# millardjn/rusty_sr

Measured on AMD Instinct MI355X. Metric: output megapixels/sec at 3x upscale (BASELINE '4x'; reference factor is hard-wired 3), higher is better.
Workload: dtype f32; 1 GPU; 1920x1080 RGB x3 upscale per GPU, imagenet.rsr, rgba8 in/out resident in HBM; io=rgba8, factor=3, parallelism=rowband1, precision=f32

## Files before the change

rusty_sr_amd/csrc/sr_kernels.hip:

```cpp
#include <hip/hip_runtime.h>
#include <stddef.h>
#include <stdint.h>

#include <mutex>
#include <set>
#include <type_traits>
#include <utility>

#include "sr_kernels.h"

#pragma clang fp contract(off)

typedef float f32x2 __attribute__((ext_vector_type(2)));
struct f32p { float x, y; };
__device__ __forceinline__ f32p operator+(f32p a, f32p b) { return f32p{a.x + b.x, a.y + b.y}; }
__device__ __forceinline__ f32p operator-(f32p a, f32p b) { return f32p{a.x - b.x, a.y - b.y}; }
__device__ __forceinline__ f32p operator*(f32p a, f32p b) { return f32p{a.x * b.x, a.y * b.y}; }
__device__ __forceinline__ f32p p_fma(f32p a, f32p b, f32p c) { return f32p{__builtin_fmaf(a.x, b.x, c.x), __builtin_fmaf(a.y, b.y, c.y)}; }
__device__ __forceinline__ void store_map8(char* p, uint32_t a, uint32_t b) { *(uint2*)p = make_uint2(a, b); }
typedef float f32x4 __attribute__((ext_vector_type(4)));
typedef float f32x16 __attribute__((ext_vector_type(16)));
typedef _Float16 f16x8 __attribute__((ext_vector_type(8)));
typedef _Float16 f16x2 __attribute__((ext_vector_type(2)));

template <int PREC>
constexpr bool kPlanar = PREC == 1;
template <int PREC, bool FINAL>
constexpr bool kH16 = PREC == 1 && !FINAL;

namespace {

constexpr int kThreads = 256;
constexpr int kTW = 32;
constexpr int kChunkFloats = 1024;
constexpr int kRingSlots = 5;
constexpr int kRingAhead = 4;
constexpr int kRingBytes = kRingSlots * 4096;

__device__ __forceinline__ float belu(float v, float beta) {
    return __fadd_rn(__fadd_rn(__fmul_rn(beta, v), __builtin_amdgcn_sqrtf(__fadd_rn(__fmul_rn(v, v), 1.0f))), -1.0f);
}

__device__ __forceinline__ f32x2 belu2(f32x2 v, float beta) {
    const f32x2 one = {1.0f, 1.0f};
    const f32x2 t = v * v + one;
    const f32x2 s = {__builtin_amdgcn_sqrtf(t.x), __builtin_amdgcn_sqrtf(t.y)};
    const f32x2 b = {beta, beta};
    return (b * v + s) - one;
}

__device__ __forceinline__ f32p split_value(f32p accm, f32p accx) {
    return p_fma(accx, f32p{1.0f / 2048.0f, 1.0f / 2048.0f}, accm);
}
__device__ __forceinline__ f32p belu2_fused2(f32p v, f32p beta) {
    const f32p one = {1.0f, 1.0f};
    const f32p t = p_fma(v, v, one);
    const f32p s = {__builtin_amdgcn_sqrtf(t.x), __builtin_amdgcn_sqrtf(t.y)};
    return p_fma(beta, v, s) - one;
}

__device__ __forceinline__ void store_belu_tile(float* base, const f32x16& acc, float bias, float beta) {
#pragma unroll
    for (int r = 0; r < 16; r += 2) {
        const f32x2 bb = {bias, bias};
        const f32x2 o = belu2(f32x2{acc[r], acc[r + 1]} + bb, beta);
        const int row = (r & 3) + 8 * (r >> 2);
        base[row * 32] = o.x;
        base[(row + 1) * 32] = o.y;
    }
}

__device__ __forceinline__ void store_belu_tile_lds(float* grow, float* stage, const f32x16& acc, float bias, float beta, int lane) {
    float* sp = stage + (4 * (lane >> 5)) * 32 + (lane & 31);
#pragma unroll
    for (int r = 0; r < 16; r += 2) {
        const f32x2 bb = {bias, bias};
        const f32x2 o = belu2(f32x2{acc[r], acc[r + 1]} + bb, beta);
        const int row = (r & 3) + 8 * (r >> 2);
        sp[row * 32] = o.x;
        sp[(row + 1) * 32] = o.y;
    }
    const f32x4* lp = (const f32x4*)stage + lane;
    const f32x4 v0 = lp[0], v1 = lp[64], v2 = lp[128], v3 = lp[192];
    f32x4* gp = (f32x4*)grow + lane;
    gp[0] = v0; gp[64] = v1; gp[128] = v2; gp[192] = v3;
}

__device__ __forceinline__ int xcd_remap(int bid, int nblk) {
    const int q = nblk >> 3, r = nblk & 7, xcd = bid & 7, idx = bid >> 3;
    return (xcd < r ? xcd * (q + 1) : r * (q + 1) + (xcd - r) * q) + idx;
}

__device__ __forceinline__ int tile_div(int t, TileDiv d) {
    return (int)((__umulhi((uint32_t)t, d.m) + (uint32_t)t) >> d.s);
}

__device__ __forceinline__ void tile_coords(const TileGrid& g, int tiles_x, int t, int& n, int& tx, int& ty) {
    const int tpi = tiles_x * g.tiles_y;
    n = tile_div(t, g.div_tpi);
    const int r = t - n * tpi;
    if (g.bw == 0) {
        ty = tile_div(r, g.div_tx);
        tx = r - ty * tiles_x;
    } else {
        int b = tile_div(r, g.div_blk);
        if (b > g.nfull) b = g.nfull;
        const int rr = r - b * g.bw * g.tiles_y;
        const bool full = b < g.nfull;
        const int w = full ? g.bw : tiles_x - g.nfull * g.bw;
        ty = full ? tile_div(rr, g.div_bw) : tile_div(rr, g.div_rem);
        tx = b * g.bw + (rr - ty * w);
    }
}

__device__ __forceinline__ float load_img(const void* img, int img_ch, bool u8, size_t px, int c) {
    if (u8) return __fdiv_rn((float)((const uint8_t*)img)[px * img_ch + c], 255.0f);
    return ((const float*)img)[px * 3 + c];
}

constexpr float kLoScale = 2048.0f;
typedef __fp16 fp16x2_t __attribute__((ext_vector_type(2)));

__device__ __forceinline__ void split_half2(f32p v, uint32_t& hi2, uint32_t& lo2) {
    const fp16x2_t h = __builtin_amdgcn_cvt_pkrtz(v.x, v.y);
    const f32p hf = {(float)h.x, (float)h.y};
    const f32p r = (v - hf) * f32p{kLoScale, kLoScale};
    hi2 = __builtin_bit_cast(uint32_t, h);
    lo2 = __builtin_bit_cast(uint32_t, __builtin_amdgcn_cvt_pkrtz(r.x, r.y));
}

typedef unsigned short u16x2 __attribute__((ext_vector_type(2)));
__device__ __forceinline__ void domain_track(uint32_t& dom, uint32_t hi2) {
    dom = __builtin_bit_cast(uint32_t, __builtin_elementwise_max(__builtin_bit_cast(u16x2, dom), __builtin_bit_cast(u16x2, hi2 & 0x7fff7fffu)));
}
__device__ __forceinline__ void domain_report(uint32_t dom, int* flag) {
    if (((dom & 0xffffu) >= 0x7bffu) | ((dom >> 16) >= 0x7bffu)) *(volatile int*)flag = 1;
}

__device__ __forceinline__ void store_belu_tile_split_cr(char* base, const f32x16& accm, const f32x16& accx, const f32x4 (&beta)[4], bool write,
                                                         long group_stride, long lo_off, uint32_t& dom) {
#pragma unroll
    for (int j = 0; j < 4; ++j) {
        const int r = 4 * j;
        const f32p v01 = belu2_fused2(split_value(f32p{accm[r], accm[r + 1]}, f32p{accx[r], accx[r + 1]}), f32p{beta[j][0], beta[j][1]});
        const f32p v23 = belu2_fused2(split_value(f32p{accm[r + 2], accm[r + 3]}, f32p{accx[r + 2], accx[r + 3]}), f32p{beta[j][2], beta[j][3]});
        uint32_t h01, l01, h23, l23;
        split_half2(v01, h01, l01);
        split_half2(v23, h23, l23);
        domain_track(dom, h01);
        domain_track(dom, h23);
        if (write) {
            store_map8(base + j * group_stride, h01, h23);
            store_map8(base + j * group_stride + lo_off, l01, l23);
        }
    }
}

template <typename F>
__device__ __forceinline__ void for_each_acc_row(F&& f) {
#pragma unroll
    for (int r = 0; r < 16; ++r) f(r, (r & 3) + 8 * (r >> 2));
}

}

__device__ __forceinline__ const char* uniform_ptr(const void* p) {
    const uint64_t v = (uint64_t)(uintptr_t)p;
    const uint32_t lo = __builtin_amdgcn_readfirstlane((uint32_t)v), hi = __builtin_amdgcn_readfirstlane((uint32_t)(v >> 32));
    return (const char*)(uintptr_t)(((uint64_t)hi << 32) | lo);
}

template <int TH, bool IMG_U8>
__global__ __launch_bounds__(kThreads, 2) void conv0_kernel(Conv0Args a) {
    constexpr int T = TH / 4;
    constexpr int TWH = kTW + 4, THH = TH + 4, NPIX = THH * TWH;
    __shared__ __attribute__((aligned(16))) float s_x[NPIX * 3 + 16];
    __shared__ __attribute__((aligned(16))) float s_w[5 * 8 * 64];

    const int tid = threadIdx.x, lane = tid & 63;
    const int wave = __builtin_amdgcn_readfirstlane(tid >> 6);
    const int i = lane & 31, h = lane >> 5;
    const int tiles_per_img = a.tiles_x * a.tiles_y;
    for (int k = tid; k < 5 * 8 * 64; k += kThreads) s_w[k] = a.wpack[k];
    if (tid < 16) s_x[NPIX * 3 + tid] = 0.f;
    if (blockIdx.x == 0 && tid < 40) a.queue_reset[tid] = (a.queue_grid[tid >> 3] - (tid & 7) + 7) >> 3;
    __shared__ float s_lut[256];
    if constexpr (IMG_U8) s_lut[tid] = __fdiv_rn((float)tid, 255.0f);
    const float bias = a.bias[i], beta = a.beta[i];
  for (int bid = blockIdx.x; bid < a.n_tiles; bid += gridDim.x) {
    const int n = tile_div(bid, a.div_tpi), t = bid - n * tiles_per_img;
    const int ty = tile_div(t, a.div_tx), tx = t - ty * a.tiles_x;
    const int x0 = tx * kTW, y0 = a.y_begin + ty * TH;
    const size_t img_px0 = (size_t)n * a.H * a.W;

    __syncthreads();
    for (int p = tid; p < NPIX; p += kThreads) {
        const int py = p / TWH, px = p - py * TWH;
        const int gy = y0 - 2 + py, gx = x0 - 2 + px;
        f32x4 v = {0.f, 0.f, 0.f, 0.f};
        if (gy >= 0 && gy < a.H && gx >= 0 && gx < a.W) {
            const size_t gp = img_px0 + (size_t)gy * a.W + gx;
            if constexpr (IMG_U8) {
                const uint8_t* q = (const uint8_t*)a.img + gp * a.img_ch;
                v.x = s_lut[q[0]]; v.y = s_lut[q[1]]; v.z = s_lut[q[2]];
            } else {
                v.x = load_img(a.img, a.img_ch, false, gp, 0);
                v.y = load_img(a.img, a.img_ch, false, gp, 1);
                v.z = load_img(a.img, a.img_ch, false, gp, 2);
            }
        }
        s_x[p * 3] = v.x; s_x[p * 3 + 1] = v.y; s_x[p * 3 + 2] = v.z;
    }
    __syncthreads();

    f32x16 acc[T];
#pragma unroll
    for (int m = 0; m < T; ++m)
#pragma unroll
        for (int r = 0; r < 16; ++r) acc[m][r] = 0.f;

    const float* xa = s_x + ((wave * T) * TWH + i) * 3 + h;
    const float* wb = s_w + (h * 32 + i) * 2;
#pragma unroll
    for (int ky = 0; ky < 5; ++ky) {
#pragma unroll
        for (int jj = 0; jj < 4; ++jj) {
            const f32x2 b = *(const f32x2*)(wb + (ky * 4 + jj) * 128);
#pragma unroll
            for (int m = 0; m < T; ++m) {
                const float* row = xa + (m + ky) * TWH * 3;
                acc[m] = __builtin_amdgcn_mfma_f32_32x32x2f32(row[4 * jj], b.x, acc[m], 0, 0, 0);
                const float a2 = (jj == 3 && h) ? 0.0f : row[4 * jj + 2];
                acc[m] = __builtin_amdgcn_mfma_f32_32x32x2f32(a2, b.y, acc[m], 0, 0, 0);
            }
        }
    }

    const bool full_x = x0 + kTW <= a.W;
#pragma unroll
    for (int m = 0; m < T; ++m) {
        const int y = y0 + wave * T + m;
        if (y >= a.y_end) continue;
        float* base = a.dst + ((size_t)n * a.img_stride + (long)y * a.pitch + x0 + 4 * h) * 32 + i;
        if (full_x) {
            store_belu_tile(base, acc[m], bias, beta);
        } else {
            for_each_acc_row([&](int r, int row) {
                if (x0 + 4 * h + row < a.W) base[row * 32] = belu(__fadd_rn(acc[m][r], bias), beta);
            });
        }
    }
  }
}

template <int TH, bool IMG_U8>
__global__ __launch_bounds__(kThreads, 3) void conv0_split_kernel(Conv0Args a) {
    constexpr int T = TH / 4;
    constexpr int TWH = kTW + 4, THH = TH + 4, NPIX = THH * TWH;
    constexpr int NB = 7;
    __shared__ __attribute__((aligned(16))) uint32_t s_px[2][NPIX * 2];
    __shared__ uint32_t s_lut[256];
    const int tid = threadIdx.x, lane = tid & 63;
    const int wave = __builtin_amdgcn_readfirstlane(tid >> 6);
    const int i = lane & 31, h = lane >> 5;
    const int tiles_per_img = a.tiles_x * a.tiles_y;
    if (blockIdx.x == 0 && tid < 40) a.queue_reset[tid] = (a.queue_grid[tid >> 3] - (tid & 7) + 7) >> 3;
    if constexpr (IMG_U8) {
        uint32_t hi2, lo2;
        split_half2(f32p{__fdiv_rn((float)tid, 255.0f), 0.0f}, hi2, lo2);
        s_lut[tid] = (hi2 & 0xffffu) | (lo2 << 16);
    }
    __shared__ __attribute__((aligned(16))) f16x8 s_w[NB * 2 * 64];
    for (int k = tid; k < NB * 2 * 64; k += kThreads) s_w[k] = ((const f16x8*)a.wpack_split)[k];
    const f16x8* wl = s_w + h * 32 + i;
    uint32_t off_a[NB], off_b[NB];
#pragma unroll
    for (int b = 0; b < NB; ++b) {
        const int ta = min(4 * b + 2 * h, 24), tb = min(4 * b + 2 * h + 1, 24);
        off_a[b] = (uint32_t)(((ta / 5) * TWH + ta % 5) * 8);
        off_b[b] = (uint32_t)(((tb / 5) * TWH + tb % 5) * 8);
    }
    const char* abase = (const char*)&s_px[0][0] + ((wave * T) * TWH + i) * 8;
    constexpr uint32_t LO = NPIX * 2 * 4;
    f32x4 bias4[4], beta4[4];
#pragma unroll
    for (int j = 0; j < 4; ++j) {
        bias4[j] = *(const f32x4*)(a.bias + 8 * j + 4 * h);
        beta4[j] = *(const f32x4*)(a.beta + 8 * j + 4 * h);
    }
    uint32_t dom = 0;
    for (int bid = blockIdx.x; bid < a.n_tiles; bid += gridDim.x) {
        const int n = tile_div(bid, a.div_tpi), t = bid - n * tiles_per_img;
        const int ty = tile_div(t, a.div_tx), tx = t - ty * a.tiles_x;
        const int x0 = tx * kTW, y0 = a.y_begin + ty * TH;
        const size_t img_px0 = (size_t)n * a.H * a.W;
        __syncthreads();
        for (int p = tid; p < NPIX; p += kThreads) {
            const int py = p / TWH, px = p - py * TWH;
            const int gy = y0 - 2 + py, gx = x0 - 2 + px;
            uint32_t h0 = 0, h1 = 0, l0 = 0, l1 = 0;
            if (gy >= 0 && gy < a.H && gx >= 0 && gx < a.W) {
                const size_t gp = img_px0 + (size_t)gy * a.W + gx;
                if constexpr (IMG_U8) {
                    const uint8_t* q = (const uint8_t*)a.img + gp * a.img_ch;
                    const uint32_t wr = s_lut[q[0]], wg = s_lut[q[1]], wb = s_lut[q[2]];
                    h0 = __builtin_amdgcn_perm(wg, wr, 0x05040100u); l0 = __builtin_amdgcn_perm(wg, wr, 0x07060302u);
                    h1 = wb & 0xffffu; l1 = wb >> 16;
                } else {
                    const float* q = (const float*)a.img + gp * 3;
                    split_half2(f32p{q[0], q[1]}, h0, l0);
                    split_half2(f32p{q[2], 0.0f}, h1, l1);
                    domain_track(dom, h0);
                    domain_track(dom, h1);
                }
            }
            *(uint2*)&s_px[0][p * 2] = make_uint2(h0, h1);
            *(uint2*)&s_px[1][p * 2] = make_uint2(l0, l1);
        }
        __syncthreads();

        f32x16 accm[T], accx[T];
#pragma unroll
        for (int m = 0; m < T; ++m)
#pragma unroll
            for (int r = 0; r < 16; ++r) { accm[m][r] = bias4[r >> 2][r & 3]; accx[m][r] = 0.f; }
#pragma unroll
        for (int b = 0; b < NB; ++b) {
            const f16x8 bh = wl[(b * 2 + 0) * 64], bl = wl[(b * 2 + 1) * 64];
#pragma unroll
            for (int m = 0; m < T; ++m) {
                const char* ra = abase + off_a[b] + m * TWH * 8;
                const char* rb = abase + off_b[b] + m * TWH * 8;
                const uint2 ha = *(const uint2*)ra, hb2 = *(const uint2*)rb;
                const uint2 la = *(const uint2*)(ra + LO), lb2 = *(const uint2*)(rb + LO);
                const uint32_t ahw[4] = {ha.x, ha.y, hb2.x, hb2.y}, alw[4] = {la.x, la.y, lb2.x, lb2.y};
                const f16x8 ah = __builtin_bit_cast(f16x8, ahw), al = __builtin_bit_cast(f16x8, alw);
                accm[m] = __builtin_amdgcn_mfma_f32_32x32x16_f16(bh, ah, accm[m], 0, 0, 0);
                accx[m] = __builtin_amdgcn_mfma_f32_32x32x16_f16(bl, ah, accx[m], 0, 0, 0);
                accx[m] = __builtin_amdgcn_mfma_f32_32x32x16_f16(bh, al, accx[m], 0, 0, 0);
            }
        }

        const bool full_x = x0 + kTW <= a.W;
#pragma unroll
        for (int m = 0; m < T; ++m) {
            const int y = y0 + wave * T + m;
            if (y >= a.y_end) continue;
            char* base = (char*)(a.dst + ((size_t)n * a.img_stride + (long)y * a.pitch) * 32) + (size_t)(x0 + i) * 16 + 8 * h;
            store_belu_tile_split_cr(base, accm[m], accx[m], beta4, full_x || x0 + i < a.W, (long)a.pitch * 16, (long)a.pitch * 64, dom);
        }
    }
    domain_report(dom, a.domain);
}

template <int TH, int KS>
struct TileGeom {
    static constexpr int R = KS / 2;
    static constexpr int TWH = kTW + 2 * R;
    static constexpr int THH = TH + 2 * R;
    static constexpr int NPIX = THH * TWH;
    static constexpr int NG = (NPIX + 63) / 64;
    static constexpr int PLANE = NG * 64 * 16;
};

template <int IMM>
__device__ __forceinline__ void lds_dma16(const void* base, uint32_t voff, uint32_t lds) {
    asm volatile("s_mov_b32 m0, %0\n\ts_nop 3\n\tglobal_load_lds_dwordx4 %1, %2 offset:%3"
                 :: "s"(lds), "v"(voff), "s"(base), "n"(IMM) : "memory");
}
__device__ __forceinline__ void lds_dma16_at(const void* base, uint32_t byte_off, uint32_t voff, uint32_t lds) {
    const uint64_t b = (uint64_t)(uintptr_t)base;
    asm volatile("s_add_u32 vcc_lo, %0, %2\n\ts_addc_u32 vcc_hi, %1, 0\n\ts_mov_b32 m0, %3\n\ts_nop 0\n\tglobal_load_lds_dwordx4 %4, vcc offset:0"
                 :: "s"((uint32_t)b), "s"((uint32_t)(b >> 32)), "s"(__builtin_amdgcn_readfirstlane(byte_off)), "s"(__builtin_amdgcn_readfirstlane(lds)), "v"(voff)
                 : "vcc", "scc", "memory");
}
__device__ __forceinline__ uint32_t lds_addr(const void* p) {
    return (uint32_t)(uintptr_t)(const __attribute__((address_space(3))) char*)p;
}

template <int TH, int KS, int NW = 4>
struct TileOffsets {
    using G = TileGeom<TH, KS>;
    static constexpr int N = (G::NG + NW - 1) / NW;
    uint32_t v[N];
    template <int PREC>
    __device__ __forceinline__ void init(int pitch, int wave, int lane) {
#pragma unroll
        for (int gi = 0; gi < N; ++gi) {
            const int P = min((wave + NW * gi) * 64 + lane, G::NPIX - 1);
            const int prow = P / G::TWH, pcol = P - prow * G::TWH;
            v[gi] = kPlanar<PREC> ? (uint32_t)(prow * pitch) * 128u + (uint32_t)pcol * 16u : (uint32_t)(prow * pitch + pcol) * 128u;
        }
    }
};

template <int TH, int KS, int PREC, int NW = 4>
__device__ __forceinline__ void stage_tile(char* tile, const float* __restrict__ src, const TileOffsets<TH, KS, NW>& off,
                                           long img_stride, int pitch, int n, int y0, int x0, int wave, int ) {
    using G = TileGeom<TH, KS>;
    const char* origin = kPlanar<PREC> ? uniform_ptr((const char*)(src + ((size_t)n * img_stride + (long)(y0 - G::R) * pitch) * 32) + (long)(x0 - G::R) * 16)
                                       : uniform_ptr(src + ((size_t)n * img_stride + (long)(y0 - G::R) * pitch + (x0 - G::R)) * 32);
#pragma unroll
    for (int gi = 0; gi < TileOffsets<TH, KS, NW>::N; ++gi) {
        const int g = wave + NW * gi;
        if (g < G::NG) {
            const uint32_t dst = __builtin_amdgcn_readfirstlane(lds_addr(tile) + g * 1024);
            if constexpr (kPlanar<PREC>) {
#pragma unroll
                for (int c = 0; c < 8; ++c) lds_dma16_at(origin, (uint32_t)(c * pitch * 16), off.v[gi], dst + c * G::PLANE);
            } else {
#define SR_DMA16(c) lds_dma16<(c) * 16>(origin, off.v[gi], dst + (c) * (G::PLANE - 16))
                SR_DMA16(0); SR_DMA16(1); SR_DMA16(2); SR_DMA16(3); SR_DMA16(4); SR_DMA16(5); SR_DMA16(6); SR_DMA16(7);
#undef SR_DMA16
            }
        }
    }
}

__device__ __forceinline__ void weight_chunk_async(char* ring_slot, const float* __restrict__ chunk,
                                                   int wave, int lane) {
    lds_dma16<0>(uniform_ptr((const char*)chunk + wave * 1024), (uint32_t)(lane * 16),
                 __builtin_amdgcn_readfirstlane(lds_addr(ring_slot) + wave * 1024));
}

template <int PENDING>
__device__ __forceinline__ void ring_barrier() {
    static_assert(PENDING >= 0 && PENDING <= 3, "");
    if constexpr (PENDING == 3) asm volatile("s_waitcnt vmcnt(3) lgkmcnt(0)" ::: "memory");
    else if constexpr (PENDING == 2) asm volatile("s_waitcnt vmcnt(2) lgkmcnt(0)" ::: "memory");
    else if constexpr (PENDING == 1) asm volatile("s_waitcnt vmcnt(1) lgkmcnt(0)" ::: "memory");
    else asm volatile("s_waitcnt vmcnt(0) lgkmcnt(0)" ::: "memory");
    __builtin_amdgcn_s_barrier();
    asm volatile("" ::: "memory");
}

__device__ __forceinline__ void ring_request(char* ring, const float* __restrict__ wpack, int gtap, int slot,
                                             int ntaps_total, int wave, int lane) {
    if (gtap + kRingAhead < ntaps_total) {
        int s2 = slot + kRingAhead;
        if (s2 >= kRingSlots) s2 -= kRingSlots;
        weight_chunk_async(ring + s2 * 4096, wpack + (size_t)(gtap + kRingAhead) * kChunkFloats, wave, lane);
    }
}
template <int EXTRA = 0>
__device__ __forceinline__ void ring_advance(int& gtap, int& slot, int ntaps_total) {
    const int pending = max(0, min(kRingAhead - 1 - EXTRA, ntaps_total - 2 - EXTRA - gtap));
    ++gtap;
    slot = slot == kRingSlots - 1 ? 0 : slot + 1;
    if (pending >= 3) ring_barrier<3>();
    else if (pending == 2) ring_barrier<2>();
    else if (pending == 1) ring_barrier<1>();
    else ring_barrier<0>();
}

template <int ABID>
__device__ __forceinline__ f32x4 mfma_quad(float w, float p, f32x4 c) { return __builtin_amdgcn_mfma_f32_4x4x1f32(w, p, c, 4, ABID, 0); }
template <int FACTOR>
constexpr int quad_groups(int nt) {
    const int ntr = FACTOR * FACTOR - 10 * nt < 10 ? FACTOR * FACTOR - 10 * nt : 10, tl = ntr - 1;
    return (16 * (tl / 5) + 3 * (tl % 5) + 2) / 4 + 1;
}
typedef f32x4 QuadAcc[8];
template <int H, int NG>
__device__ __forceinline__ void quad_rank1(QuadAcc& acc, float w, float p) {
    if constexpr (NG > 0) acc[0] = mfma_quad<8 * H + 0>(w, p, acc[0]);
    if constexpr (NG > 1) acc[1] = mfma_quad<8 * H + 1>(w, p, acc[1]);
    if constexpr (NG > 2) acc[2] = mfma_quad<8 * H + 2>(w, p, acc[2]);
    if constexpr (NG > 3) acc[3] = mfma_quad<8 * H + 3>(w, p, acc[3]);
    if constexpr (NG > 4) acc[4] = mfma_quad<8 * H + 4>(w, p, acc[4]);
    if constexpr (NG > 5) acc[5] = mfma_quad<8 * H + 5>(w, p, acc[5]);
// ... 1174 lines not shown
        }
        st.issued += 3 * PER;
        seq = st.issued;
    }
    __device__ __forceinline__ void store_split(char* s_hi, int lo_off, const uint32_t* s_lut2, float scale, int tid, const StepStream& st) {
        wait_vm(st.issued - seq);
#pragma unroll
        for (int k = 0; k < PER; ++k)
#pragma unroll
            for (int ch = 0; ch < 3; ++ch) asm volatile("" : "+v"(raw[k][ch]));
#pragma unroll
        for (int k = 0; k < PER; ++k) {
            const int p = tid + 256 * k;
            if (p < NPIX) {
                if constexpr (IMG_U8) lin_split_store_u8(s_hi, lo_off, p, s_lut2[raw[k][0]], s_lut2[raw[k][1]], s_lut2[raw[k][2]]);
                else lin_split_store_f32(s_hi, lo_off, p, __uint_as_float(raw[k][0]), __uint_as_float(raw[k][1]), __uint_as_float(raw[k][2]), scale);
            }
        }
    }
    __device__ __forceinline__ void store(float* s_x, const float* s_lut, int tid, const StepStream& st) {
        wait_vm(st.issued - seq);
#pragma unroll
        for (int k = 0; k < PER; ++k)
#pragma unroll
            for (int ch = 0; ch < 3; ++ch) asm volatile("" : "+v"(raw[k][ch]));
#pragma unroll
        for (int k = 0; k < PER; ++k) {
            const int p = tid + 256 * k;
            if (p < NPIX) {
                f32x4 v;
                if constexpr (IMG_U8) {
                    v.x = s_lut[raw[k][0]]; v.y = s_lut[raw[k][1]]; v.z = s_lut[raw[k][2]];
                } else {
                    v.x = __uint_as_float(raw[k][0]); v.y = __uint_as_float(raw[k][1]); v.z = __uint_as_float(raw[k][2]);
                }
                v.w = 0.f;
                *(f32x4*)&s_x[p * 4] = v;
            }
        }
    }
};

struct QueueState {
    uint32_t pulled;
    uint32_t heads;
    int seq_pull, seq_snap;
    int own;
};
__device__ __forceinline__ void queue_pull_async(const StageArgs& a, int xcd, int wave, int lane, StepStream& st, QueueState& qs) {
    if (wave != 0) return;
    if (lane == 0) {
        const int* p = a.queue + xcd;
        asm volatile("global_atomic_add %0, %1, %2, off sc0" : "=v"(qs.pulled) : "v"(p), "v"(1u) : "memory");
    }
    qs.seq_pull = ++st.issued;
}
__device__ __forceinline__ void queue_presolve(const StageArgs& a, int xcd, int wave, int lane, StepStream& st, QueueState& qs) {
    if (wave != 0) return;
    wait_vm(st.issued - qs.seq_pull);
    asm volatile("" : "+v"(qs.pulled));
    const int idx = __builtin_amdgcn_readfirstlane((int)qs.pulled);
    qs.own = queue_slot(xcd, a.grid[0].ntiles, a.grid[1].ntiles, idx);
    if (qs.own < 0) {
        const int* p = a.queue + (lane & 7);
        asm volatile("global_load_dword %0, %1, off sc1" : "=v"(qs.heads) : "v"(p) : "memory");
        qs.seq_snap = ++st.issued;
    }
}
__device__ __forceinline__ void queue_publish(const StageArgs& a, int xcd, int wave, int lane, StepStream& st, QueueState& qs, volatile int* mailbox) {
    if (wave != 0) return;
    int t = qs.own;
    if (t < 0) {
        const int nbig = a.grid[0].ntiles, nsmall = a.grid[1].ntiles;
        wait_vm(st.issued - qs.seq_snap);
        asm volatile("" : "+v"(qs.heads));
        for (int k = 1; k < 8 && t < 0; ++k) {
            const int x = (xcd + k) & 7;
            if ((int)__builtin_amdgcn_readlane((int)qs.heads, x) >= queue_total(x, nbig, nsmall)) continue;
            int j = 0;
            if (lane == 0) j = atomicAdd(&a.queue[x], 1);
            t = queue_slot(x, nbig, nsmall, __builtin_amdgcn_readfirstlane(j));
        }
    }
    if (lane == 0) *mailbox = t;
    asm volatile("s_waitcnt lgkmcnt(0)" ::: "memory");
}

struct NoHook { __device__ __forceinline__ void operator()() const {} };
template <int PREC, int KSN, typename Hook = NoHook>
struct PipeStream {
    StepStream& st;
    const HalfRequest& rq;
    const HalfTile<KSN>& htn;
    const StageArgs& a;
    uint32_t ring_lds;
    const char* wbase;
    int gs0;
    int wave, lane;
    volatile int* mailbox;
    int xcd;
    QueueState& qs;
    int snap_step;
    int step_no;
    Hook last_step_hook;
    __device__ __forceinline__ void begin_step() {
        step_request(st, gs0 + step_no, ring_lds, wbase, lane);
        if (mailbox && step_no == snap_step) queue_presolve(a, xcd, wave, lane, st, qs);
        ++step_no;
    }
    __device__ __forceinline__ void piece(int g) {
        if (g < HalfTile<KSN>::G::NG && g < rq.ng) {
            htn.stage_one(g, rq.origin, rq.dst);
            st.tile_seq = ++st.issued;
        }
    }
    __device__ __forceinline__ int slot() const { return st.slot; }
    template <int EXTRA> __device__ __forceinline__ void end_step(bool last) {
        if (last) last_step_hook();
        if (last && mailbox) queue_publish(a, xcd, wave, lane, st, qs, mailbox);
        step_advance<EXTRA>(st, last, PREC == 1 && gs0 + step_no <= kRingAhead);
    }
};

template <int NSRC, int KS0, bool FINAL, bool IMG_U8, bool OUT_U8, int PREC, int FACTOR = 3, bool WINO = false, int W3H = 0>
__global__ __launch_bounds__(256, 2) void conv_stage_pipe_kernel(StageArgs a) {
    static_assert(!WINO || (NSRC <= 2 && KS0 == 5 && !FINAL && PREC == 0), "WINO: stages 1 and 2 of the exact mode");
    static_assert(W3H >= 0 && W3H <= 2 && (W3H == 0 || (WINO && NSRC == 2)), "W3H: the first W3H halves of stage 2's 3x3 source as Winograd rows");
    __builtin_amdgcn_s_setprio(3);
    constexpr int NTN = FINAL ? (FACTOR * FACTOR + 9) / 10 : 1;
    using H0 = HalfTile<KS0>;
    using H3 = HalfTile<3>;
    constexpr int HB = H0::BYTES;
    constexpr int NH = 2 * NSRC;
    constexpr bool H16 = kH16<PREC, FINAL>;
    constexpr int NSTEPS = WINO ? 2 * kWinoSteps + (NSRC - 1) * (W3H * kWino3Steps + (2 - W3H) * H3::STEPS)
                         : H16 ? KS0 * KS0 + (NSRC - 1) * 9
                               : 2 * (H0::STEPS + (NSRC - 1) * H3::STEPS) * NTN;
    extern __shared__ __attribute__((aligned(16))) char smem[];
    char* ring = smem + 2 * HB;
    volatile int* s_next = (volatile int*)(ring + kRingBytes);
    float* s_wlin = (float*)(ring + kRingBytes + 16);
    float* s_lut = s_wlin + 9 * NTN * 128;
    constexpr bool kLinOwn = FINAL && NTN == 1;
    float* s_xown = s_lut + 256;
    const uint32_t lds0 = lds_addr(smem);

    const int tid = threadIdx.x, lane = tid & 63;
    const int wave = __builtin_amdgcn_readfirstlane(tid >> 6);
    const int i = lane & 31;
    const int nbig = a.grid[0].ntiles, nsmall = a.grid[1].ntiles;
    const int xcd = blockIdx.x & 7;
    const uint32_t ring_lds = __builtin_amdgcn_readfirstlane(lds_addr(ring) + wave * 1024);
    const char* wbase = uniform_ptr((const char*)a.wpack + wave * 1024);
    float bias[NTN];
#pragma unroll
    for (int nt = 0; nt < NTN; ++nt) bias[nt] = a.bias[nt * 32 + i];
    const float beta = FINAL ? 0.f : a.beta[i];
    f32x4 bias2[2], beta2[2];
#pragma unroll
    for (int ch = 0; ch < 2; ++ch) {
        bias2[ch] = H16 ? *(const f32x4*)(a.bias + 16 * ch + 4 * (lane >> 4)) : f32x4{0.f, 0.f, 0.f, 0.f};
        beta2[ch] = H16 ? *(const f32x4*)(a.beta + 16 * ch + 4 * (lane >> 4)) : f32x4{0.f, 0.f, 0.f, 0.f};
    }
    constexpr bool kFinalT = FINAL && PREC == 1;
    f32x4 fbias[kFinalT ? NTN : 1][4];
    if constexpr (kFinalT) {
#pragma unroll
        for (int nt = 0; nt < NTN; ++nt)
#pragma unroll
            for (int k = 0; k < 4; ++k) fbias[nt][k] = *(const f32x4*)(a.bias + 32 * nt + 16 * (lane >> 5) + 4 * k);
    }
    constexpr bool kQuad = FINAL && PREC == 0;
    float qbias[kQuad ? 3 * FACTOR * FACTOR : 1];
    if constexpr (kQuad) {
#pragma unroll
        for (int ch = 0; ch < 3 * FACTOR * FACTOR; ++ch) {
            const int tr = ch / 3, tl = tr % 10;
            qbias[ch] = a.bias[(tr / 10) * 32 + 16 * (tl / 5) + 3 * (tl % 5) + ch % 3];
        }
    }
    H0 h0;
    H3 h3;
    h0.template init<PREC>(a.pitch, lane);
    if constexpr (NSRC >= 2) h3.template init<PREC>(a.pitch, lane);

    typedef const uint32_t __attribute__((address_space(4)))* KernWords;
    static_assert(sizeof(TileGrid) == 64 && offsetof(StageArgs, grid) % 4 == 0, "TileGrid is read as 16 dwords");
    auto coords = [&](int t, int& n, int& x0, int& y0, bool& small) {
        KernWords kw = (KernWords)__builtin_amdgcn_kernarg_segment_ptr();
        asm volatile("" : "+s"(kw));
        int tx, ty;
        small = t >= nbig;
        uint32_t words[16];
#pragma unroll
        for (int k = 0; k < 16; ++k) words[k] = kw[offsetof(StageArgs, grid) / 4 + (small ? 16 : 0) + k];
        TileGrid g;
        __builtin_memcpy(&g, words, sizeof(g));
        tile_coords(g, a.tiles_x, small ? t - nbig : t, n, tx, ty);
        y0 = g.y0 + ty * (small ? 4 : 8);
        x0 = tx * kTW;
    };

    if constexpr (FINAL) {
        const float* wlin = a.wpack + (size_t)NSTEPS * kChunkFloats;
        for (int k = tid; k < (PREC == 1 ? 3 * NTN * 256 : 9 * NTN * 128); k += 256) s_wlin[k] = wlin[k];
        if constexpr (IMG_U8) s_lut[tid] = PREC == 1 ? __uint_as_float(lin_split_table_entry(tid, 4.0f * FACTOR * FACTOR)) : __fdiv_rn((float)tid, 255.0f);
    }
    const int first = queue_first(blockIdx.x, nbig, nsmall);
    if (first < 0) return;
    const bool single = (int)gridDim.x >= nbig + nsmall;
    int n, x0, y0;
    bool small;
    coords(first, n, x0, y0, small);
    h0.template stage<PREC>(lds0, a.src[0], 0, a.img_stride, a.pitch, n, y0, x0, wave);
#pragma unroll
    for (int k = 0; k < kRingAhead; ++k) weight_chunk_async(ring + k * 4096, a.wpack + k * kChunkFloats, wave, lane);
    constexpr int NG0 = H0::G::NG;
    StepStream st{0, NSTEPS, false, NG0 + kRingAhead, {0, NG0 + 2, NG0 + 3, NG0 + 4}, NG0};
    static_assert(kRingAhead == 4, "q[] initialiser");
    wait_vm_barrier<true>(st.issued - (NG0 + 1 + (PREC == 1 ? 1 : 0)));

    int nn = 0, nx0 = 0, ny0 = 0;
    bool nsmall_tile = false;
    uint32_t dom = 0;

    auto tile_body = [&](auto tc) {
        constexpr int T = decltype(tc)::value;
        constexpr int TH = 4 * T;
        f32x16 acc[NTN * T], accx[PREC == 1 ? NTN * T : 1];
#pragma unroll
        for (int m = 0; m < NTN * T; ++m)
#pragma unroll
            for (int r = 0; r < 16; ++r) {
                acc[m][r] = (PREC == 1 && !FINAL) ? bias[0] : 0.f;
                if constexpr (PREC == 1) accx[m][r] = 0.f;
            }
        f32x4 qm[H16 ? T : 1][2][2], qx[H16 ? T : 1][2][2];
        if constexpr (H16) {
#pragma unroll
            for (int m = 0; m < T; ++m)
#pragma unroll
                for (int k = 0; k < 4; ++k) { qm[m][k >> 1][k & 1] = bias2[k & 1]; qx[m][k >> 1][k & 1] = f32x4{0.f, 0.f, 0.f, 0.f}; }
        }
        constexpr bool QUAD = FINAL && PREC == 0 && T == 2;
        QuadAcc qa[QUAD ? NTN : 1];
        if constexpr (QUAD) {
#pragma unroll
            for (int nt = 0; nt < NTN; ++nt)
#pragma unroll
                for (int g = 0; g < 8; ++g) qa[nt][g] = f32x4{0.f, 0.f, 0.f, 0.f};
        }
        constexpr int NWACC = WINO ? 3 + NSRC : 1;
        f32x16 wacc[NWACC];
#pragma unroll
        for (int p = 0; p < NWACC; ++p)
#pragma unroll
            for (int r = 0; r < 16; ++r) wacc[p][r] = 0.f;
        QueueState qs{0u, 0u, 0, 0, -1};
        if (!single) queue_pull_async(a, xcd, wave, lane, st, qs);
        st.have_next = false;
        LinPrefetch<IMG_U8, TH> linpx;
        auto do_half = [&](auto jc) {
            constexpr int j = decltype(jc)::value;
            constexpr int src = j >> 1;
            constexpr int KSJ = src == 0 ? KS0 : 3;
            constexpr int KSN = (j + 1 < NH) ? (((j + 1) >> 1) == 0 ? KS0 : 3) : KS0;
            const uint32_t other = lds0 + ((j + 1) & 1) * HB;
            const char* hb = smem + (j & 1) * HB;
            if constexpr (j == 1) {
                const int next = single ? -1 : __builtin_amdgcn_readfirstlane(*s_next);
                st.have_next = next >= 0;
                if (st.have_next) coords(next, nn, nx0, ny0, nsmall_tile);
            }
            HalfRequest rq;
            if constexpr (j + 1 < NH)
                rq = HalfRequest{T == 2 ? HalfTile<KSN>::G::NG : HalfTile<KSN>::NG_SMALL,
                                 HalfTile<KSN>::template origin_of<PREC>(a.src[(j + 1) >> 1], (j + 1) & 1, a.img_stride, a.pitch, n, y0, x0, wave),
                                 HalfTile<KSN>::plane_of(other, wave)};
            else
                rq = HalfRequest{!st.have_next ? 0 : nsmall_tile ? HalfTile<KSN>::NG_SMALL : HalfTile<KSN>::G::NG,
                                 HalfTile<KSN>::template origin_of<PREC>(a.src[0], 0, a.img_stride, a.pitch, nn, ny0, nx0, wave),
                                 HalfTile<KSN>::plane_of(other, wave)};
            if constexpr (FINAL && j == (kLinOwn ? NH - 2 : NH - 1)) linpx.issue(a, n, y0, x0, tid, st);
            const HalfTile<KSN>* htn;
            if constexpr (KSN == KS0) htn = (const HalfTile<KSN>*)&h0; else htn = (const HalfTile<KSN>*)&h3;
            using GJ = TileGeom<8, KSJ>;
            constexpr int PAIRS_J = (KSJ * KSJ - 1) / 2;
            constexpr bool WINO3_J = WINO && src == 1 && (j & 1) < W3H;
            constexpr int STEPS_J = WINO ? (src == 0 ? kWinoSteps : WINO3_J ? kWino3Steps : H3::STEPS) : H16 ? PAIRS_J + (j & 1) : HalfTile<KSJ>::STEPS * NTN;
            constexpr int GS0 = WINO ? (j < 2 ? j * kWinoSteps : 2 * kWinoSteps + (j - 2) * (W3H >= 1 ? kWino3Steps : H3::STEPS)) : H16 ? (src == 0 ? 0 : KS0 * KS0 + (src - 1) * 9) + (j & 1) * PAIRS_J
                                    : (j == 0 ? 0 : j == 1 ? H0::STEPS : 2 * H0::STEPS + (j - 2) * H3::STEPS) * NTN;
            constexpr int LIN_LO_J = LinPrefetch<IMG_U8, TH>::NPIX * 8;
            auto lin_store = [&]() {
                if constexpr (kLinOwn && j == NH - 2) {
                    if constexpr (PREC == 1) linpx.store_split((char*)s_xown, LIN_LO_J, (const uint32_t*)s_lut, 4.0f * FACTOR * FACTOR, tid, st);
                    else linpx.store(s_xown, s_lut, tid, st);
                    asm volatile("s_waitcnt lgkmcnt(0)" ::: "memory");
                }
            };
            PipeStream<PREC, KSN, decltype(lin_store)> sm{st, rq, *htn, a, ring_lds, wbase, GS0, wave, lane, (j == 0 && !single) ? s_next : nullptr, xcd, qs, STEPS_J > 3 ? STEPS_J - 3 : 0, 0, lin_store};
            if constexpr (WINO && src == 0) half_steps_wino<GJ::TWH, GJ::PLANE, T, KS0>(wacc, hb, ring, sm, wave, lane);
            else if constexpr (WINO3_J) half_steps_wino<GJ::TWH, GJ::PLANE, T, 3>(wacc, hb, ring, sm, wave, lane);
            else if constexpr (WINO) half_steps_pairs<GJ::TWH, GJ::PLANE, T>(wacc, hb, ring, sm, wave, lane);
            else if constexpr (QUAD) half_steps_f32<GJ::TWH, GJ::PLANE, KSJ, T, NTN, true, FACTOR>(qa, hb, ring, sm, wave, lane);
            else if constexpr (PREC == 0) half_steps_f32<GJ::TWH, GJ::PLANE, KSJ, T, NTN>(acc, hb, ring, sm, wave, lane);
            else if constexpr (H16) half_steps_h16<GJ::TWH, GJ::PLANE, 2, KSJ, T, (j & 1) != 0, -HB>(qm, qx, hb, ring, sm, wave, lane);
            else half_steps_h<GJ::TWH, GJ::PLANE, 2, KSJ, T, NTN>(acc, accx, hb, ring, sm, wave, lane);
        };
        do_half(std::integral_constant<int, 0>{});
        do_half(std::integral_constant<int, 1>{});
        if constexpr (NH > 2) { do_half(std::integral_constant<int, 2>{}); do_half(std::integral_constant<int, 3>{}); }
        if constexpr (NH > 4) { do_half(std::integral_constant<int, 4>{}); do_half(std::integral_constant<int, 5>{}); }
        if constexpr (FINAL) {
            constexpr int LIN_LO = LinPrefetch<IMG_U8, TH>::NPIX * 8;
            float* s_x = kLinOwn ? s_xown : (float*)(smem + HB);
            if constexpr (!kLinOwn) {
                if constexpr (PREC == 1) linpx.store_split((char*)s_x, LIN_LO, (const uint32_t*)s_lut, 4.0f * FACTOR * FACTOR, tid, st);
                else linpx.store(s_x, s_lut, tid, st);
                asm volatile("s_waitcnt lgkmcnt(0)" ::: "memory");
                __builtin_amdgcn_s_barrier();
                asm volatile("" ::: "memory");
            }
            if constexpr (PREC == 1) lin_mfma_h<TH, T, NTN>(acc, accx, (const char*)s_x, LIN_LO, (const f16x8*)s_wlin, wave, lane);
            else if constexpr (QUAD) lin_mfma_quad<NTN, FACTOR>(qa, s_x, s_wlin, wave, lane);
            else lin_mfma<TH, T, NTN>(acc, s_x, s_wlin, wave, lane);
            if constexpr (!kLinOwn) {
                asm volatile("s_waitcnt lgkmcnt(0)" ::: "memory");
                __builtin_amdgcn_s_barrier();
                asm volatile("" ::: "memory");
            }
        }
        int stores;
        if constexpr (H16) stores = stage_epilogue_h16<T>(a, qm, qx, beta2, n, x0, y0, wave, lane, dom);
        else if constexpr (QUAD) stores = stage_epilogue_quad<NTN, OUT_U8, FACTOR>(a, qa, qbias, n, x0, y0, wave, lane);
        else if constexpr (kFinalT) stores = stage_epilogue_final_t<T, NTN, OUT_U8, FACTOR>(a, acc, accx, fbias, n, x0, y0, wave, lane);
        else {
            float* scratch = FINAL ? nullptr : (float*)(smem + ((NH - 1) & 1) * HB + wave * H0::G::PLANE);
            if constexpr (WINO) stores = stage_epilogue_wino<T, NWACC>(a, wacc, bias[0], beta, n, x0, y0, wave, lane, scratch);
            else stores = stage_epilogue<TH, T, NTN, FINAL, OUT_U8, FACTOR>(a, acc, bias, beta, n, x0, y0, wave, lane, scratch);
        }
        if constexpr (PREC == 1) st.issued += stores;
    };

    constexpr bool kBigTiles = !(FINAL && FACTOR == 4 && PREC == 1);
    int budget = nbig + nsmall;
    while (true) {
        if constexpr (kBigTiles) {
            if (small) tile_body(std::integral_constant<int, 1>{});
            else tile_body(std::integral_constant<int, 2>{});
        } else {
            if (!small) __builtin_trap();
            tile_body(std::integral_constant<int, 1>{});
        }
        if (!st.have_next) break;
        if (--budget <= 0) {
            asm volatile("s_waitcnt vmcnt(0)" ::: "memory");
            __builtin_trap();
        }
        n = nn; x0 = nx0; y0 = ny0; small = nsmall_tile;
    }
    if constexpr (PREC == 1 && !FINAL) domain_report(dom, a.domain);
}


__global__ __launch_bounds__(256) void clear_borders_kernel(ClearArgs a) {
    float4* m = reinterpret_cast<float4*>(a.map[blockIdx.y]);
    const long rows_per = a.img_stride / a.pitch;
    const long row = blockIdx.x;
    const long base = row * a.pitch;
    long end = base + a.pitch;
// ... 154 lines not shown
```

Baseline: 5320 output MP/s.

## Issue first-tile pixel and bias/weight loads early to overlap kernel prologue latency

In both conv0 kernels, each block loads its first tile's raw pixels into registers before the weight, LUT and bias setup, then converts and writes them to LDS afterwards, so global-load latency overlaps the prologue. In the stage kernel, the bias and final-layer weight loads move after the early-exit check and are issued before the first tile staging and weight-ring prefetch. Their LDS stores and register uses are deferred, with asm barriers forcing the loads to land at a chosen point. This shortens the serial latency chain at kernel start, at the cost of more registers for prefetched data and duplicated first-tile handling code.

```diff
diff --git a/rusty_sr_amd/csrc/sr_kernels.hip b/rusty_sr_amd/csrc/sr_kernels.hip
--- a/rusty_sr_amd/csrc/sr_kernels.hip
+++ b/rusty_sr_amd/csrc/sr_kernels.hip
@@ -171,28 +171,85 @@
 }
 
 template <int TH, bool IMG_U8>
+struct Conv0Pixels {
+    static constexpr int TWH = kTW + 4, NPIX = (TH + 4) * TWH, PER = (NPIX + kThreads - 1) / kThreads;
+    uint32_t raw[PER][3];
+    __device__ __forceinline__ void load(const Conv0Args& a, int n, int y0, int x0, int tid) {
+#pragma unroll
+        for (int k = 0; k < PER; ++k) {
+            const int p = min(tid + kThreads * k, NPIX - 1);
+            const int py = p / TWH, px = p - py * TWH;
+            const int gy = min(max(y0 - 2 + py, 0), a.H - 1), gx = min(max(x0 - 2 + px, 0), a.W - 1);
+            const size_t gp = (size_t)n * a.H * a.W + (size_t)gy * a.W + gx;
+#pragma unroll
+            for (int c = 0; c < 3; ++c) {
+                if constexpr (IMG_U8) raw[k][c] = ((const uint8_t*)a.img)[gp * a.img_ch + c];
+                else raw[k][c] = __float_as_uint(((const float*)a.img)[gp * 3 + c]);
+            }
+        }
+    }
+    static __device__ __forceinline__ bool inside(const Conv0Args& a, int y0, int x0, int p) {
+        const int py = p / TWH, px = p - py * TWH;
+        const int gy = y0 - 2 + py, gx = x0 - 2 + px;
+        return gy >= 0 && gy < a.H && gx >= 0 && gx < a.W;
+    }
+};
+__device__ __forceinline__ void conv0_tile(const Conv0Args& a, int th, int bid, int& n, int& x0, int& y0) {
+    n = tile_div(bid, a.div_tpi);
+    const int t = bid - n * a.tiles_x * a.tiles_y;
+    const int ty = tile_div(t, a.div_tx), tx = t - ty * a.tiles_x;
+    x0 = tx * kTW;
+    y0 = a.y_begin + ty * th;
+}
+
+template <int TH, bool IMG_U8>
 __global__ __launch_bounds__(kThreads, 2) void conv0_kernel(Conv0Args a) {
     constexpr int T = TH / 4;
     constexpr int TWH = kTW + 4, THH = TH + 4, NPIX = THH * TWH;
+    using Px = Conv0Pixels<TH, IMG_U8>;
     __shared__ __attribute__((aligned(16))) float s_x[NPIX * 3 + 16];
     __shared__ __attribute__((aligned(16))) float s_w[5 * 8 * 64];
 
     const int tid = threadIdx.x, lane = tid & 63;
     const int wave = __builtin_amdgcn_readfirstlane(tid >> 6);
     const int i = lane & 31, h = lane >> 5;
-    const int tiles_per_img = a.tiles_x * a.tiles_y;
+    Px first;
+    const bool has_tile = (int)blockIdx.x < a.n_tiles;
+    if (has_tile) {
+        int n, x0, y0;
+        conv0_tile(a, TH, blockIdx.x, n, x0, y0);
+        first.load(a, n, y0, x0, tid);
+    }
     for (int k = tid; k < 5 * 8 * 64; k += kThreads) s_w[k] = a.wpack[k];
     if (tid < 16) s_x[NPIX * 3 + tid] = 0.f;
     if (blockIdx.x == 0 && tid < 40) a.queue_reset[tid] = (a.queue_grid[tid >> 3] - (tid & 7) + 7) >> 3;
     __shared__ float s_lut[256];
     if constexpr (IMG_U8) s_lut[tid] = __fdiv_rn((float)tid, 255.0f);
     const float bias = a.bias[i], beta = a.beta[i];
+    auto put = [&](int p, bool in, uint32_t r, uint32_t g, uint32_t b) {
+        f32x4 v = {0.f, 0.f, 0.f, 0.f};
+        if (in) {
+            if constexpr (IMG_U8) { v.x = s_lut[r]; v.y = s_lut[g]; v.z = s_lut[b]; }
+            else { v.x = __uint_as_float(r); v.y = __uint_as_float(g); v.z = __uint_as_float(b); }
+        }
+        s_x[p * 3] = v.x; s_x[p * 3 + 1] = v.y; s_x[p * 3 + 2] = v.z;
+    };
+    if (has_tile) {
+        int n, x0, y0;
+        conv0_tile(a, TH, blockIdx.x, n, x0, y0);
+        __syncthreads();
+#pragma unroll
+        for (int k = 0; k < Px::PER; ++k) {
+            const int p = tid + kThreads * k;
+            if (p < NPIX) put(p, Px::inside(a, y0, x0, p), first.raw[k][0], first.raw[k][1], first.raw[k][2]);
+        }
+    }
   for (int bid = blockIdx.x; bid < a.n_tiles; bid += gridDim.x) {
-    const int n = tile_div(bid, a.div_tpi), t = bid - n * tiles_per_img;
-    const int ty = tile_div(t, a.div_tx), tx = t - ty * a.tiles_x;
-    const int x0 = tx * kTW, y0 = a.y_begin + ty * TH;
+    int n, x0, y0;
+    conv0_tile(a, TH, bid, n, x0, y0);
     const size_t img_px0 = (size_t)n * a.H * a.W;
 
+    if (bid != (int)blockIdx.x) {
     __syncthreads();
     for (int p = tid; p < NPIX; p += kThreads) {
         const int py = p / TWH, px = p - py * TWH;
@@ -211,6 +268,7 @@
         }
         s_x[p * 3] = v.x; s_x[p * 3 + 1] = v.y; s_x[p * 3 + 2] = v.z;
     }
+    }
     __syncthreads();
 
     f32x16 acc[T];
@@ -263,7 +321,14 @@
     const int tid = threadIdx.x, lane = tid & 63;
     const int wave = __builtin_amdgcn_readfirstlane(tid >> 6);
     const int i = lane & 31, h = lane >> 5;
-    const int tiles_per_img = a.tiles_x * a.tiles_y;
+    using Px = Conv0Pixels<TH, IMG_U8>;
+    Px first;
+    const bool has_tile = (int)blockIdx.x < a.n_tiles;
+    if (has_tile) {
+        int n, x0, y0;
+        conv0_tile(a, TH, blockIdx.x, n, x0, y0);
+        first.load(a, n, y0, x0, tid);
+    }
     if (blockIdx.x == 0 && tid < 40) a.queue_reset[tid] = (a.queue_grid[tid >> 3] - (tid & 7) + 7) >> 3;
     if constexpr (IMG_U8) {
         uint32_t hi2, lo2;
@@ -289,33 +354,56 @@
         beta4[j] = *(const f32x4*)(a.beta + 8 * j + 4 * h);
     }
     uint32_t dom = 0;
+    auto put = [&](int p, bool in, uint32_t r, uint32_t g, uint32_t b) {
+        uint32_t h0 = 0, h1 = 0, l0 = 0, l1 = 0;
+        if (in) {
+            if constexpr (IMG_U8) {
+                const uint32_t wr = s_lut[r], wg = s_lut[g], wb = s_lut[b];
+                h0 = __builtin_amdgcn_perm(wg, wr, 0x05040100u); l0 = __builtin_amdgcn_perm(wg, wr, 0x07060302u);
+                h1 = wb & 0xffffu; l1 = wb >> 16;
+            } else {
+                split_half2(f32p{__uint_as_float(r), __uint_as_float(g)}, h0, l0);
+                split_half2(f32p{__uint_as_float(b), 0.0f}, h1, l1);
+                domain_track(dom, h0);
+                domain_track(dom, h1);
+            }
+        }
+        *(uint2*)&s_px[0][p * 2] = make_uint2(h0, h1);
+        *(uint2*)&s_px[1][p * 2] = make_uint2(l0, l1);
+    };
+    if (has_tile) {
+        int n, x0, y0;
+        conv0_tile(a, TH, blockIdx.x, n, x0, y0);
+        __syncthreads();
+#pragma unroll
+        for (int k = 0; k < Px::PER; ++k) {
+            const int p = tid + kThreads * k;
+            if (p < NPIX) put(p, Px::inside(a, y0, x0, p), first.raw[k][0], first.raw[k][1], first.raw[k][2]);
+        }
+    }
     for (int bid = blockIdx.x; bid < a.n_tiles; bid += gridDim.x) {
-        const int n = tile_div(bid, a.div_tpi), t = bid - n * tiles_per_img;
-        const int ty = tile_div(t, a.div_tx), tx = t - ty * a.tiles_x;
-        const int x0 = tx * kTW, y0 = a.y_begin + ty * TH;
+        int n, x0, y0;
+        conv0_tile(a, TH, bid, n, x0, y0);
         const size_t img_px0 = (size_t)n * a.H * a.W;
-        __syncthreads();
-        for (int p = tid; p < NPIX; p += kThreads) {
-            const int py = p / TWH, px = p - py * TWH;
-            const int gy = y0 - 2 + py, gx = x0 - 2 + px;
-            uint32_t h0 = 0, h1 = 0, l0 = 0, l1 = 0;
-            if (gy >= 0 && gy < a.H && gx >= 0 && gx < a.W) {
-                const size_t gp = img_px0 + (size_t)gy * a.W + gx;
-                if constexpr (IMG_U8) {
-                    const uint8_t* q = (const uint8_t*)a.img + gp * a.img_ch;
-                    const uint32_t wr = s_lut[q[0]], wg = s_lut[q[1]], wb = s_lut[q[2]];
-                    h0 = __builtin_amdgcn_perm(wg, wr, 0x05040100u); l0 = __builtin_amdgcn_perm(wg, wr, 0x07060302u);
-                    h1 = wb & 0xffffu; l1 = wb >> 16;
-                } else {
-                    const float* q = (const float*)a.img + gp * 3;
-                    split_half2(f32p{q[0], q[1]}, h0, l0);
-                    split_half2(f32p{q[2], 0.0f}, h1, l1);
-                    domain_track(dom, h0);
-                    domain_track(dom, h1);
+        if (bid != (int)blockIdx.x) {
+            __syncthreads();
+            for (int p = tid; p < NPIX; p += kThreads) {
+                const int py = p / TWH, px = p - py * TWH;
+                const int gy = y0 - 2 + py, gx = x0 - 2 + px;
+                const bool in = gy >= 0 && gy < a.H && gx >= 0 && gx < a.W;
+                uint32_t r = 0, g = 0, b = 0;
+                if (in) {
+                    const size_t gp = img_px0 + (size_t)gy * a.W + gx;
+                    if constexpr (IMG_U8) {
+                        const uint8_t* q = (const uint8_t*)a.img + gp * a.img_ch;
+                        r = q[0]; g = q[1]; b = q[2];
+                    } else {
+                        const float* q = (const float*)a.img + gp * 3;
+                        r = __float_as_uint(q[0]); g = __float_as_uint(q[1]); b = __float_as_uint(q[2]);
+                    }
                 }
-            }
-            *(uint2*)&s_px[0][p * 2] = make_uint2(h0, h1);
-            *(uint2*)&s_px[1][p * 2] = make_uint2(l0, l1);
+                put(p, in, r, g, b);
+            }
         }
         __syncthreads();
 
@@ -1796,37 +1884,6 @@
     const int xcd = blockIdx.x & 7;
     const uint32_t ring_lds = __builtin_amdgcn_readfirstlane(lds_addr(ring) + wave * 1024);
     const char* wbase = uniform_ptr((const char*)a.wpack + wave * 1024);
-    float bias[NTN];
-#pragma unroll
-    for (int nt = 0; nt < NTN; ++nt) bias[nt] = a.bias[nt * 32 + i];
-    const float beta = FINAL ? 0.f : a.beta[i];
-    f32x4 bias2[2], beta2[2];
-#pragma unroll
-    for (int ch = 0; ch < 2; ++ch) {
-        bias2[ch] = H16 ? *(const f32x4*)(a.bias + 16 * ch + 4 * (lane >> 4)) : f32x4{0.f, 0.f, 0.f, 0.f};
-        beta2[ch] = H16 ? *(const f32x4*)(a.beta + 16 * ch + 4 * (lane >> 4)) : f32x4{0.f, 0.f, 0.f, 0.f};
-    }
-    constexpr bool kFinalT = FINAL && PREC == 1;
-    f32x4 fbias[kFinalT ? NTN : 1][4];
-    if constexpr (kFinalT) {
-#pragma unroll
-        for (int nt = 0; nt < NTN; ++nt)
-#pragma unroll
-            for (int k = 0; k < 4; ++k) fbias[nt][k] = *(const f32x4*)(a.bias + 32 * nt + 16 * (lane >> 5) + 4 * k);
-    }
-    constexpr bool kQuad = FINAL && PREC == 0;
-    float qbias[kQuad ? 3 * FACTOR * FACTOR : 1];
-    if constexpr (kQuad) {
-#pragma unroll
-        for (int ch = 0; ch < 3 * FACTOR * FACTOR; ++ch) {
-            const int tr = ch / 3, tl = tr % 10;
-            qbias[ch] = a.bias[(tr / 10) * 32 + 16 * (tl / 5) + 3 * (tl % 5) + ch % 3];
-        }
-    }
-    H0 h0;
-    H3 h3;
-    h0.template init<PREC>(a.pitch, lane);
-    if constexpr (NSRC >= 2) h3.template init<PREC>(a.pitch, lane);
 
     typedef const uint32_t __attribute__((address_space(4)))* KernWords;
     static_assert(sizeof(TileGrid) == 64 && offsetof(StageArgs, grid) % 4 == 0, "TileGrid is read as 16 dwords");
@@ -1845,21 +1902,81 @@
         x0 = tx * kTW;
     };
 
-    if constexpr (FINAL) {
-        const float* wlin = a.wpack + (size_t)NSTEPS * kChunkFloats;
-        for (int k = tid; k < (PREC == 1 ? 3 * NTN * 256 : 9 * NTN * 128); k += 256) s_wlin[k] = wlin[k];
-        if constexpr (IMG_U8) s_lut[tid] = PREC == 1 ? __uint_as_float(lin_split_table_entry(tid, 4.0f * FACTOR * FACTOR)) : __fdiv_rn((float)tid, 255.0f);
-    }
     const int first = queue_first(blockIdx.x, nbig, nsmall);
     if (first < 0) return;
-    const bool single = (int)gridDim.x >= nbig + nsmall;
+    float bias[NTN];
+#pragma unroll
+    for (int nt = 0; nt < NTN; ++nt) bias[nt] = a.bias[nt * 32 + i];
+    float beta = FINAL ? 0.f : a.beta[i];
+    f32x4 bias2[2], beta2[2];
+#pragma unroll
+    for (int ch = 0; ch < 2; ++ch) {
+        bias2[ch] = H16 ? *(const f32x4*)(a.bias + 16 * ch + 4 * (lane >> 4)) : f32x4{0.f, 0.f, 0.f, 0.f};
+        beta2[ch] = H16 ? *(const f32x4*)(a.beta + 16 * ch + 4 * (lane >> 4)) : f32x4{0.f, 0.f, 0.f, 0.f};
+    }
+    constexpr bool kFinalT = FINAL && PREC == 1;
+    f32x4 fbias[kFinalT ? NTN : 1][4];
+    if constexpr (kFinalT) {
+#pragma unroll
+        for (int nt = 0; nt < NTN; ++nt)
+#pragma unroll
+            for (int k = 0; k < 4; ++k) fbias[nt][k] = *(const f32x4*)(a.bias + 32 * nt + 16 * (lane >> 5) + 4 * k);
+    }
+    constexpr bool kQuad = FINAL && PREC == 0;
+    float qbias[kQuad ? 3 * FACTOR * FACTOR : 1];
+    if constexpr (kQuad) {
+#pragma unroll
+        for (int ch = 0; ch < 3 * FACTOR * FACTOR; ++ch) {
+            const int tr = ch / 3, tl = tr % 10;
+            qbias[ch] = a.bias[(tr / 10) * 32 + 16 * (tl / 5) + 3 * (tl % 5) + ch % 3];
+        }
+    }
+    constexpr int NW4 = FINAL ? (PREC == 1 ? 3 * NTN * 256 : 9 * NTN * 128) / 4 : 0, NWI = FINAL ? (NW4 + 255) / 256 : 1;
+    static_assert(!FINAL || (PREC == 1 ? 3 * NTN * 256 : 9 * NTN * 128) % 4 == 0, "the fixed weights are copied 16 bytes at a time");
+    f32x4 w4[NWI];
+    if constexpr (FINAL) {
+        const f32x4* wlin = (const f32x4*)(a.wpack + (size_t)NSTEPS * kChunkFloats);
+#pragma unroll
+        for (int k = 0; k < NWI; ++k) w4[k] = wlin[min(tid + 256 * k, NW4 - 1)];
+    }
+
     int n, x0, y0;
     bool small;
     coords(first, n, x0, y0, small);
+    H0 h0;
+    H3 h3;
+    h0.template init<PREC>(a.pitch, lane);
     h0.template stage<PREC>(lds0, a.src[0], 0, a.img_stride, a.pitch, n, y0, x0, wave);
 #pragma unroll
     for (int k = 0; k < kRingAhead; ++k) weight_chunk_async(ring + k * 4096, a.wpack + k * kChunkFloats, wave, lane);
+    if constexpr (NSRC >= 2) h3.template init<PREC>(a.pitch, lane);
+
+    if constexpr (FINAL) {
+#pragma unroll
+        for (int k = 0; k < NWI; ++k)
+            if (tid + 256 * k < NW4) ((f32x4*)s_wlin)[tid + 256 * k] = w4[k];
+        if constexpr (IMG_U8) s_lut[tid] = PREC == 1 ? __uint_as_float(lin_split_table_entry(tid, 4.0f * FACTOR * FACTOR)) : __fdiv_rn((float)tid, 255.0f);
+    }
+#define SR_LANDED(v) asm volatile("" : "+v"(v))
+    if constexpr (H16) {
+        SR_LANDED(bias2[0]); SR_LANDED(bias2[1]); SR_LANDED(beta2[0]); SR_LANDED(beta2[1]);
+    } else if constexpr (kFinalT) {
+#pragma unroll
+        for (int nt = 0; nt < NTN; ++nt)
+#pragma unroll
+            for (int k = 0; k < 4; ++k) SR_LANDED(fbias[nt][k]);
+    } else {
+#pragma unroll
+        for (int nt = 0; nt < NTN; ++nt) SR_LANDED(bias[nt]);
+        if constexpr (!FINAL) SR_LANDED(beta);
+    }
+    if constexpr (kQuad) {
+#pragma unroll
+        for (int ch = 0; ch < 3 * FACTOR * FACTOR; ++ch) SR_LANDED(qbias[ch]);
+    }
+#undef SR_LANDED
     constexpr int NG0 = H0::G::NG;
+    const bool single = (int)gridDim.x >= nbig + nsmall;
     StepStream st{0, NSTEPS, false, NG0 + kRingAhead, {0, NG0 + 2, NG0 + 3, NG0 + 4}, NG0};
     static_assert(kRingAhead == 4, "q[] initialiser");
     wait_vm_barrier<true>(st.issued - (NG0 + 1 + (PREC == 1 ? 1 : 0)));
```

Result: no change. 5316 output MP/s (-0.1%).
